# stanfordnlp/mac-network

Hardware: NVIDIA H100
Metric: mac_reasoning_steps_per_sec (higher is better)
Workload: dtype bf16

## Files before the change

mac_network_b200/csrc/read_step.cuh:

```cuda
#pragma once
#include "tc_gemm.cuh"

namespace mac {

constexpr int RS_D = 512;
constexpr int RS_BM = 64;
constexpr int RS_KB = RS_D / TC_BK;
constexpr int RS_BLK = RS_BM * TC_BK * 2;
constexpr int RS_A_BYTES = RS_KB * RS_BLK;
constexpr int RS_B_HALF = 256 * TC_BK * 2;
constexpr int RS_CONSUMERS = 256;
constexpr int RS_THREADS = RS_CONSUMERS + 32;

constexpr int RS128_BM = 128;
constexpr int RS128_BLK = RS128_BM * TC_BK * 2;
constexpr int RS128_A_BYTES = RS_KB * RS128_BLK;
constexpr int RS128_STAGE = RS_B_HALF;
constexpr int RS128_STAGES = 3;
constexpr int RS128_Q0 = RS_KB;
constexpr int RS128_G1B = RS128_Q0 + 2;
constexpr int RS128_Q1 = RS128_G1B + RS_KB;
constexpr int RS128_G2A = RS128_Q1 + 2;
constexpr int RS128_G2B = RS128_G2A + RS_KB;
constexpr int RS128_SLOTS = RS128_G2B + RS_KB;
constexpr int RS128_CONSUMERS = 256;
constexpr int RS128_THREADS = RS128_CONSUMERS + 128;
constexpr int RS128_SMEM_BYTES = RS128_A_BYTES + RS128_STAGES * RS128_STAGE + 1024  +
                                 8 * (RS_KB + 2 * RS128_STAGES) ;
static_assert(RS128_SMEM_BYTES <= 232448, "over the sm_90 per-block shared memory opt-in limit");
static_assert(RS128_BLK % 1024 == 0 && RS128_STAGE % 1024 == 0 && (RS128_BM / 2) * 128 % 1024 == 0,
              "swizzled operands need 1024-byte alignment");
static_assert(2 * RS128_BLK == RS128_STAGE, "a ring slot holds two Q blocks");
constexpr int RS128_PRODUCER_REGS = 40;
constexpr int RS128_CONSUMER_REGS = 232;
static_assert(RS128_PRODUCER_REGS + 2 * RS128_CONSUMER_REGS <= 3 * (65536 / RS128_THREADS / 8 * 8), "register budget");

__device__ __forceinline__ float bf16lo(uint32_t w) { return __uint_as_float(w << 16); }
__device__ __forceinline__ float bf16hi(uint32_t w) { return __uint_as_float(w & 0xffff0000u); }

__device__ __forceinline__ void wgmma_bf16_n256(float (&d)[128], uint64_t adesc, uint64_t bdesc, uint32_t accum) {
  asm volatile(
      "{\n\t.reg .pred p;\n\t"
      "setp.ne.b32 p, %130, 0;\n\t"
      "wgmma.mma_async.sync.aligned.m64n256k16.f32.bf16.bf16 "
      "{%0, %1, %2, %3, %4, %5, %6, %7, %8, %9, %10, %11, %12, %13, %14, %15, %16, %17, %18, %19, %20, %21, %22, %23, %24, %25, %26, %27, %28, %29, %30, %31, %32, %33, %34, %35, %36, %37, %38, %39, %40, %41, %42, %43, %44, %45, %46, %47, %48, %49, %50, %51, %52, %53, %54, %55, %56, %57, %58, %59, %60, %61, %62, %63, %64, %65, %66, %67, %68, %69, %70, %71, %72, %73, %74, %75, %76, %77, %78, %79, %80, %81, %82, %83, %84, %85, %86, %87, %88, %89, %90, %91, %92, %93, %94, %95, %96, %97, %98, %99, %100, %101, %102, %103, %104, %105, %106, %107, %108, %109, %110, %111, %112, %113, %114, %115, %116, %117, %118, %119, %120, %121, %122, %123, %124, %125, %126, %127}, %128, %129, p, 1, 1, 0, 0;\n\t}"
      : "+f"(d[0]), "+f"(d[1]), "+f"(d[2]), "+f"(d[3]), "+f"(d[4]), "+f"(d[5]), "+f"(d[6]), "+f"(d[7]), "+f"(d[8]), "+f"(d[9]), "+f"(d[10]), "+f"(d[11]), "+f"(d[12]), "+f"(d[13]), "+f"(d[14]), "+f"(d[15]), "+f"(d[16]), "+f"(d[17]), "+f"(d[18]), "+f"(d[19]), "+f"(d[20]), "+f"(d[21]), "+f"(d[22]), "+f"(d[23]), "+f"(d[24]), "+f"(d[25]), "+f"(d[26]), "+f"(d[27]), "+f"(d[28]), "+f"(d[29]), "+f"(d[30]), "+f"(d[31]), "+f"(d[32]), "+f"(d[33]), "+f"(d[34]), "+f"(d[35]), "+f"(d[36]), "+f"(d[37]), "+f"(d[38]), "+f"(d[39]), "+f"(d[40]), "+f"(d[41]), "+f"(d[42]), "+f"(d[43]), "+f"(d[44]), "+f"(d[45]), "+f"(d[46]), "+f"(d[47]), "+f"(d[48]), "+f"(d[49]), "+f"(d[50]), "+f"(d[51]), "+f"(d[52]), "+f"(d[53]), "+f"(d[54]), "+f"(d[55]), "+f"(d[56]), "+f"(d[57]), "+f"(d[58]), "+f"(d[59]), "+f"(d[60]), "+f"(d[61]), "+f"(d[62]), "+f"(d[63]), "+f"(d[64]), "+f"(d[65]), "+f"(d[66]), "+f"(d[67]), "+f"(d[68]), "+f"(d[69]), "+f"(d[70]), "+f"(d[71]), "+f"(d[72]), "+f"(d[73]), "+f"(d[74]), "+f"(d[75]), "+f"(d[76]), "+f"(d[77]), "+f"(d[78]), "+f"(d[79]), "+f"(d[80]), "+f"(d[81]), "+f"(d[82]), "+f"(d[83]), "+f"(d[84]), "+f"(d[85]), "+f"(d[86]), "+f"(d[87]), "+f"(d[88]), "+f"(d[89]), "+f"(d[90]), "+f"(d[91]), "+f"(d[92]), "+f"(d[93]), "+f"(d[94]), "+f"(d[95]), "+f"(d[96]), "+f"(d[97]), "+f"(d[98]), "+f"(d[99]), "+f"(d[100]), "+f"(d[101]), "+f"(d[102]), "+f"(d[103]), "+f"(d[104]), "+f"(d[105]), "+f"(d[106]), "+f"(d[107]), "+f"(d[108]), "+f"(d[109]), "+f"(d[110]), "+f"(d[111]), "+f"(d[112]), "+f"(d[113]), "+f"(d[114]), "+f"(d[115]), "+f"(d[116]), "+f"(d[117]), "+f"(d[118]), "+f"(d[119]), "+f"(d[120]), "+f"(d[121]), "+f"(d[122]), "+f"(d[123]), "+f"(d[124]), "+f"(d[125]), "+f"(d[126]), "+f"(d[127])
      : "l"(adesc), "l"(bdesc), "r"(accum));
}
inline bool read_step_supported(int B, int N, int d) {
  return d == RS_D && N >= 1 && N <= 256 && B >= 1 && B < (1 << 22);
}

struct ReadStepParams {
  int M, N;
  const float* y;
  const float* ctrl;
  const float* bm2;
  const float* wr;
  float* logits;
};

__device__ __forceinline__ void rs_consumer_bar() { asm volatile("bar.sync 1, %0;" ::"n"(RS_CONSUMERS) : "memory"); }

__device__ __forceinline__ void rs128_wg_bar(int g) { asm volatile("bar.sync %0, 128;" ::"r"(1 + g) : "memory"); }

__device__ __forceinline__ void rs128_gemm_half(float (&acc)[128], uint32_t a_u, uint32_t ring_u, uint64_t* full,
                                                uint64_t* empty, int t0, int lane) {
  for (int j = 0; j < RS_KB; ++j) {
    const int t = t0 + j, s = t % RS128_STAGES;
    mbar_wait(&full[s], (t / RS128_STAGES) & 1);
    const uint64_t adesc = make_sw128_kmajor_desc(a_u + j * RS128_BLK);
    const uint64_t bdesc = make_sw128_kmajor_desc(ring_u + s * RS128_STAGE);
    wgmma_fence();
#pragma unroll
    for (int k = 0; k < TC_BK / 16; ++k) wgmma_bf16_n256(acc, adesc + 2 * k, bdesc + 2 * k, (j || k) ? 1u : 0u);
    wgmma_commit();
    wgmma_wait<1>();
    wgmma_hold(acc);
    if (j && lane == 0) mbar_arrive(&empty[(t - 1) % RS128_STAGES]);
  }
  wgmma_wait<0>();
  wgmma_hold(acc);
  if (lane == 0) mbar_arrive(&empty[(t0 + RS_KB - 1) % RS128_STAGES]);
}

__device__ __forceinline__ int rs128_sw_off(int r, int n, int blk) {
  return (n >> 6) * blk + r * 128 + ((((n & 63) >> 3) ^ (r & 7)) << 4) + (n & 7) * 2;
}

__global__ void __launch_bounds__(RS128_THREADS, 1)
read_step_kernel(const __grid_constant__ CUtensorMap map_p, const __grid_constant__ CUtensorMap map_q,
                 const __grid_constant__ CUtensorMap map_w1, const __grid_constant__ CUtensorMap map_w2,
                 const ReadStepParams p) {
  extern __shared__ unsigned char smem_dyn[];
  const uint32_t base_u32 = smem_u32(smem_dyn);
  unsigned char* a_tile = smem_dyn + ((1024u - (base_u32 & 1023u)) & 1023u);
  unsigned char* ring = a_tile + RS128_A_BYTES;
  uint64_t* pfull = reinterpret_cast<uint64_t*>(ring + RS128_STAGES * RS128_STAGE);
  uint64_t* full = pfull + RS_KB;
  uint64_t* empty = full + RS128_STAGES;

  const int warp = threadIdx.x >> 5, lane = threadIdx.x & 31;
  const int row0 = blockIdx.x * RS128_BM;

  if (threadIdx.x == RS128_CONSUMERS) {
    tma_prefetch_desc(&map_p);
    tma_prefetch_desc(&map_q);
    tma_prefetch_desc(&map_w1);
    tma_prefetch_desc(&map_w2);
    for (int i = 0; i < RS_KB; ++i) mbar_init(&pfull[i], 1);
    for (int i = 0; i < RS128_STAGES; ++i) {
      mbar_init(&full[i], 1);
      mbar_init(&empty[i], RS128_CONSUMERS / 32);
    }
    fence_mbar_init();
  }
  __syncthreads();

  if (warp >= RS128_CONSUMERS / 32) {
    asm volatile("setmaxnreg.dec.sync.aligned.u32 %0;" ::"n"(RS128_PRODUCER_REGS));
    if (warp == RS128_CONSUMERS / 32 && elect_one()) {
      auto load_p = [&](int j) {
        mbar_expect_tx(&pfull[j], RS128_BLK);
        tma_load_2d(a_tile + j * RS128_BLK, &map_p, j * TC_BK, row0, &pfull[j]);
      };
      for (int t = 0; t < RS128_SLOTS; ++t) {
        if (t < RS128_STAGES) load_p(t);
        else if (t == RS128_STAGES)
          for (int j = RS128_STAGES; j < RS_KB; ++j) load_p(j);
        const int s = t % RS128_STAGES;
        mbar_wait(&empty[s], ((t / RS128_STAGES) & 1) ^ 1);
        unsigned char* dst = ring + s * RS128_STAGE;
        mbar_expect_tx(&full[s], RS128_STAGE);
        if (t < RS128_G2A) {
          const int half = t >= RS128_G1B, u = t - half * RS128_G1B;
          if (u < RS_KB) {
            tma_load_2d(dst, &map_w1, u * TC_BK, 256 * half, &full[s]);
          } else {
            const int kb = 4 * half + 2 * (u - RS_KB);
            tma_load_2d(dst, &map_q, kb * TC_BK, row0, &full[s]);
            tma_load_2d(dst + RS128_BLK, &map_q, (kb + 1) * TC_BK, row0, &full[s]);
          }
        } else {
          const int half = t >= RS128_G2B, u = t - (half ? RS128_G2B : RS128_G2A);
          tma_load_2d(dst, &map_w2, u * TC_BK, 256 * half, &full[s]);
        }
      }
    }
    return;
  }

  asm volatile("setmaxnreg.inc.sync.aligned.u32 %0;" ::"n"(RS128_CONSUMER_REGS));
  const int g = warp >> 2;
  const int wt = threadIdx.x & 127;
  const int rl = 16 * (warp & 3) + (lane >> 2);
  const int cq = 2 * (lane & 3);
  const int rowg = row0 + 64 * g;
  unsigned char* a_wg = a_tile + g * (RS128_BM / 2) * 128;
  const uint32_t a_u = smem_u32(a_wg), ring_u = smem_u32(ring);
  const int prow = wt >> 3;
  const int poff = prow * 128 + (wt & 7) * 16;
  const int pcol = ((wt & 7) ^ (prow & 7)) << 3;
  int yoff[4];
#pragma unroll
  for (int u = 0; u < 4; ++u) yoff[u] = min(rowg + prow + 16 * u, p.M - 1) / p.N * RS_D + pcol;

  float acc[128];
  float4 y0[4], y1[4];
  auto load_y = [&](int j) {
#pragma unroll
    for (int u = 0; u < 4; ++u) {
      y0[u] = *reinterpret_cast<const float4*>(p.y + yoff[u] + j * TC_BK);
      y1[u] = *reinterpret_cast<const float4*>(p.y + yoff[u] + j * TC_BK + 4);
    }
  };
  load_y(0);
  for (int j = 0; j < RS_KB; ++j) {
    const int s = j % RS128_STAGES;
    mbar_wait(&pfull[j], 0);
#pragma unroll
    for (int u = 0; u < 4; ++u) {
      uint4* c = reinterpret_cast<uint4*>(a_wg + j * RS128_BLK + poff + u * 16 * 128);
      const uint4 v = *c;
      *c = make_uint4(pack_bf16(bf16lo(v.x) * y0[u].x, bf16hi(v.x) * y0[u].y), pack_bf16(bf16lo(v.y) * y0[u].z, bf16hi(v.y) * y0[u].w),
                      pack_bf16(bf16lo(v.z) * y1[u].x, bf16hi(v.z) * y1[u].y), pack_bf16(bf16lo(v.w) * y1[u].z, bf16hi(v.w) * y1[u].w));
    }
    fence_proxy_async();
    rs128_wg_bar(g);
    mbar_wait(&full[s], (j / RS128_STAGES) & 1);
    const uint64_t adesc = make_sw128_kmajor_desc(a_u + j * RS128_BLK);
    const uint64_t bdesc = make_sw128_kmajor_desc(ring_u + s * RS128_STAGE);
    wgmma_fence();
#pragma unroll
    for (int k = 0; k < TC_BK / 16; ++k) wgmma_bf16_n256(acc, adesc + 2 * k, bdesc + 2 * k, (j || k) ? 1u : 0u);
    wgmma_commit();
    if (j + 1 < RS_KB) load_y(j + 1);
    wgmma_wait<1>();
    wgmma_hold(acc);
    if (j && lane == 0) mbar_arrive(&empty[(j - 1) % RS128_STAGES]);
  }
  wgmma_wait<0>();
  wgmma_hold(acc);
  if (lane == 0) mbar_arrive(&empty[(RS_KB - 1) % RS128_STAGES]);

  uint32_t h0[64];
#pragma unroll
  for (int q = 0; q < 2; ++q) {
    const int t = RS128_Q0 + q, s = t % RS128_STAGES;
    mbar_wait(&full[s], (t / RS128_STAGES) & 1);
    const unsigned char* q_tile = ring + s * RS128_STAGE + g * (RS128_BM / 2) * 128 - 2 * q * RS128_BLK;
#pragma unroll
    for (int h = 0; h < 2; ++h) {
      const int r = rl + 8 * h;
      const bool live = rowg + r < p.M;
#pragma unroll
      for (int j = 16 * q; j < 16 * q + 16; ++j) {
        const uint32_t qv = *reinterpret_cast<const uint32_t*>(q_tile + rs128_sw_off(r, cq + 8 * j, RS128_BLK));
        h0[2 * j + h] = live ? pack_bf16(elu_fast(acc[4 * j + 2 * h] + bf16lo(qv)), elu_fast(acc[4 * j + 2 * h + 1] + bf16hi(qv)))
                             : 0u;
      }
    }
    __syncwarp();
    if (lane == 0) mbar_arrive(&empty[s]);
  }

  rs128_gemm_half(acc, a_u, ring_u, full, empty, RS128_G1B, lane);

  rs128_wg_bar(g);
#pragma unroll
  for (int h = 0; h < 2; ++h) {
    const int r = rl + 8 * h;
#pragma unroll
    for (int j = 0; j < 32; ++j) *reinterpret_cast<uint32_t*>(a_wg + rs128_sw_off(r, cq + 8 * j, RS128_BLK)) = h0[2 * j + h];
  }
#pragma unroll
  for (int q = 0; q < 2; ++q) {
    const int t = RS128_Q1 + q, s = t % RS128_STAGES;
    mbar_wait(&full[s], (t / RS128_STAGES) & 1);
    const unsigned char* q_tile = ring + s * RS128_STAGE + g * (RS128_BM / 2) * 128 - 2 * q * RS128_BLK;
#pragma unroll
    for (int h = 0; h < 2; ++h) {
      const int r = rl + 8 * h;
      const bool live = rowg + r < p.M;
#pragma unroll
      for (int j = 16 * q; j < 16 * q + 16; ++j) {
        const int n = cq + 8 * j;
        const uint32_t qv = *reinterpret_cast<const uint32_t*>(q_tile + rs128_sw_off(r, n, RS128_BLK));
        *reinterpret_cast<uint32_t*>(a_wg + rs128_sw_off(r, 256 + n, RS128_BLK)) =
            live ? pack_bf16(elu_fast(acc[4 * j + 2 * h] + bf16lo(qv)), elu_fast(acc[4 * j + 2 * h + 1] + bf16hi(qv))) : 0u;
      }
    }
    __syncwarp();
    if (lane == 0) mbar_arrive(&empty[s]);
  }
  fence_proxy_async();
  rs128_wg_bar(g);

  float part[2][2];
#pragma unroll
  for (int half = 0; half < 2; ++half) {
    rs128_gemm_half(acc, a_u, ring_u, full, empty, half ? RS128_G2B : RS128_G2A, lane);
#pragma unroll
    for (int h = 0; h < 2; ++h) {
      const int row = rowg + rl + 8 * h;
      const float* crow = p.ctrl + (size_t)(min(row, p.M - 1) / p.N) * RS_D + 256 * half;
      const float* bm2 = p.bm2 + 256 * half;
      const float* wr = p.wr + 256 * half;
      float s = 0.f;
#pragma unroll
      for (int j = 0; j < 32; ++j) {
        const int n = cq + 8 * j;
        const float2 cc = __ldg(reinterpret_cast<const float2*>(crow + n));
        const float2 bb = __ldg(reinterpret_cast<const float2*>(bm2 + n));
        const float2 ww = __ldg(reinterpret_cast<const float2*>(wr + n));
        const float t0 = elu_fast((acc[4 * j + 2 * h] + bb.x) * cc.x);
        const float t1 = elu_fast((acc[4 * j + 2 * h + 1] + bb.y) * cc.y);
        s = fmaf(t0, ww.x, s);
        s = fmaf(t1, ww.y, s);
      }
      s += __shfl_xor_sync(0xffffffffu, s, 1);
      s += __shfl_xor_sync(0xffffffffu, s, 2);
      part[half][h] = s;
    }
  }
#pragma unroll
  for (int h = 0; h < 2; ++h) {
    const int row = rowg + rl + 8 * h;
    if ((lane & 3) == 0 && row < p.M) p.logits[row] = part[0][h] + part[1][h];
  }
}

inline int read_step_launch(const void* P, const void* Q, float* logits, const void* kb_bf16, const float* y,
                            const float* control, const mac_read_weights* w, float* att, float* info, int B, int N, int d,
                            cudaStream_t stream) {
  const int M = B * N;
  CUtensorMap mp, mq, mw1, mw2;
  int st = make_tmap_2d(&mp, P, 1, (uint64_t)M, (uint64_t)d, (uint64_t)d * 2, RS128_BM, TC_BK, 1);
  if (st != MAC_OK) return st;
  st = make_tmap_2d(&mq, Q, 1, (uint64_t)M, (uint64_t)d, (uint64_t)d * 2, RS128_BM, TC_BK, 1);
  if (st != MAC_OK) return st;
  st = make_tmap_2d(&mw1, w->Wm_bf16, 1, (uint64_t)d, (uint64_t)d, (uint64_t)2 * d * 2, 256, TC_BK, 1);
  if (st != MAC_OK) return st;
  st = make_tmap_2d(&mw2, w->Wm2_bf16, 1, (uint64_t)d, (uint64_t)d, (uint64_t)d * 2, 256, TC_BK, 1);
  if (st != MAC_OK) return st;
  ReadStepParams p{};
  p.M = M; p.N = N; p.y = y; p.ctrl = control; p.bm2 = w->bm2; p.wr = w->wr; p.logits = logits;
  MAC_CUDA_TRY(cudaFuncSetAttribute(read_step_kernel, cudaFuncAttributeMaxDynamicSharedMemorySize, RS128_SMEM_BYTES));
  read_step_kernel<<<(M + RS128_BM - 1) / RS128_BM, RS128_THREADS, RS128_SMEM_BYTES, stream>>>(mp, mq, mw1, mw2, p);
  MAC_LAUNCH_CHECK();
  return mac_kb_attend_fwd(logits, 1, w->br, kb_bf16, 1, att, info, B, N, d, stream);
}

}
```

profiles/read_step_128.py:

```python
import argparse
import json
import os
import shutil
import subprocess
import sys
import tempfile

import numpy as np

ROOT = os.path.dirname(os.path.dirname(os.path.abspath(__file__)))
LIB_REL = os.path.join("mac_network_b200", "csrc", "libmac_b200.so")
SIDES = ("base", "new")


def device_info():
    q = subprocess.run(["nvidia-smi", "--query-gpu=name,power.limit,clocks.max.sm", "--format=csv,noheader"],
                       capture_output=True, text=True, timeout=60)
    name, power, clock = [s.strip() for s in q.stdout.strip().splitlines()[0].split(",")]
    return {"name": name, "power_limit": power, "max_sm_clock": clock}


def spread(xs):
    xs = [float(x) for x in xs]
    return {"median": float(np.median(xs)), "min": min(xs), "max": max(xs), "runs": [round(x, 3) for x in xs]}


def tree_copy(dst, lib):
    shutil.copytree(ROOT, dst, ignore=shutil.ignore_patterns(".git", "*.o", "__pycache__"))
    shutil.copyfile(lib, os.path.join(dst, LIB_REL))
    return dst


def bench(tree, extra, timeout_s=1800):
    out = subprocess.run([sys.executable, os.path.join(tree, "bench.py")] + extra, capture_output=True, text=True,
                         timeout=timeout_s, cwd=tree)
    if out.returncode != 0:
        raise RuntimeError("bench.py %s: exit %d: %s" % (" ".join(extra), out.returncode, out.stderr[-2000:]))
    line = json.loads(out.stdout.strip().splitlines()[-1])
    print("%s %s: %s" % (os.path.basename(tree), " ".join(extra), line.get("value", "done")), flush=True)
    return line


def main():
    ap = argparse.ArgumentParser()
    ap.add_argument("out_dir")
    ap.add_argument("--base-lib", required=True)
    ap.add_argument("--runs", type=int, default=3)
    ap.add_argument("--roof-runs", type=int, default=6)
    ap.add_argument("--part", default="both", choices=["rooflines", "headline", "both"])
    args = ap.parse_args()
    out = {"device": device_info(), "runs": args.runs, "roof_runs": args.roof_runs,
           "headline_args": "--gpus 1 --steps 480 --warmup 12 --skip-cpu"}
    tmp = tempfile.mkdtemp(prefix="read_step_128_")
    try:
        trees = {"base": tree_copy(os.path.join(tmp, "base"), os.path.abspath(args.base_lib)),
                 "new": tree_copy(os.path.join(tmp, "new"), os.path.join(ROOT, LIB_REL))}
        dumps = {s: os.path.join(tmp, "dump_" + s) for s in SIDES}

        roof = {s: [] for s in SIDES}
        for _ in range(args.roof_runs if args.part != "headline" else 0):
            for s in SIDES:
                roof[s].append(bench(trees[s], ["--rooflines-only"])["read_step_fused"]["us"])
        if args.part != "headline":
            out["read_step_fused_us"] = {s: spread(roof[s]) for s in SIDES}
            out["read_step_fused_speedup"] = (out["read_step_fused_us"]["base"]["median"] /
                                              out["read_step_fused_us"]["new"]["median"])
        if args.part == "rooflines":
            return finish(args, out)

        lines = {s: {"headline": [], "bf16_gqa": [], "batched_one_stream": [], "batched_two_streams": []} for s in SIDES}
        for i in range(args.runs):
            for s in SIDES:
                extra = ["--gpus", "1", "--steps", "480", "--warmup", "12", "--skip-cpu"]
                line = bench(trees[s], extra + (["--dump-outputs", dumps[s]] if i == 0 else []))
                lines[s]["headline"].append(line["value"])
                lines[s]["bf16_gqa"].append(line["sub_lines"]["bf16_gqa"]["value"])
                lines[s]["batched_one_stream"].append(line["info_batched_requests"]["requests_x6_one_stream"]["value"])
                lines[s]["batched_two_streams"].append(line["info_batched_requests"]["requests_x6_two_streams"]["value"])
        out["reasoning_steps_per_s"] = {s: {k: spread(v) for k, v in lines[s].items()} for s in SIDES}
        out["headline_speedup"] = (out["reasoning_steps_per_s"]["new"]["headline"]["median"] /
                                   out["reasoning_steps_per_s"]["base"]["headline"]["median"])

        same = {}
        for name in sorted(os.listdir(dumps["base"])):
            a, b = np.load(os.path.join(dumps["base"], name)), np.load(os.path.join(dumps["new"], name))
            same[name] = bool(a.shape == b.shape and a.dtype == b.dtype and a.tobytes() == b.tobytes())
        out["outputs_bit_identical"] = same
    finally:
        shutil.rmtree(tmp, ignore_errors=True)
    finish(args, out)


def finish(args, out):
    os.makedirs(args.out_dir, exist_ok=True)
    path = os.path.join(args.out_dir, "read_step_128_%s_h100.json" % args.part)
    with open(path, "w") as f:
        json.dump(out, f, indent=1)
    print(json.dumps(out))


if __name__ == "__main__":
    main()
```

Measured before the change: 19460.

## Split read-step first GEMM into N=128 quarters and overlap epilogue with next quarter

Splits the first GEMM of the fused read-step kernel into four N=128 quarters, held in two 64-register accumulators used in ping-pong. The ELU(acc+Q) epilogue of each quarter runs while the next quarter's wgmma is in flight, instead of running only after the full N=256 halves finish. The TMA ring is rebuilt as six 128-row slots, with Q blocks interleaved into the weight stream, and the second GEMM still issues N=256 by pairing adjacent slots. This adds more barrier traffic, narrower wgmma shapes in GEMM1, and higher register pressure from holding three quarters of bf16 h values.

```diff
diff --git a/mac_network_b200/csrc/read_step.cuh b/mac_network_b200/csrc/read_step.cuh
--- a/mac_network_b200/csrc/read_step.cuh
+++ b/mac_network_b200/csrc/read_step.cuh
@@ -8,21 +8,20 @@
 constexpr int RS_KB = RS_D / TC_BK;
 constexpr int RS_BLK = RS_BM * TC_BK * 2;
 constexpr int RS_A_BYTES = RS_KB * RS_BLK;
-constexpr int RS_B_HALF = 256 * TC_BK * 2;
 constexpr int RS_CONSUMERS = 256;
 constexpr int RS_THREADS = RS_CONSUMERS + 32;
 
 constexpr int RS128_BM = 128;
 constexpr int RS128_BLK = RS128_BM * TC_BK * 2;
 constexpr int RS128_A_BYTES = RS_KB * RS128_BLK;
-constexpr int RS128_STAGE = RS_B_HALF;
-constexpr int RS128_STAGES = 3;
-constexpr int RS128_Q0 = RS_KB;
-constexpr int RS128_G1B = RS128_Q0 + 2;
-constexpr int RS128_Q1 = RS128_G1B + RS_KB;
-constexpr int RS128_G2A = RS128_Q1 + 2;
-constexpr int RS128_G2B = RS128_G2A + RS_KB;
-constexpr int RS128_SLOTS = RS128_G2B + RS_KB;
+constexpr int RS128_QN = 128;
+constexpr int RS128_STAGE = RS128_QN * TC_BK * 2;
+constexpr int RS128_STAGES = 6;
+constexpr int RS128_G1Q = RS_KB;
+constexpr int RS128_G1Q_SLOTS = RS_KB + 2;
+constexpr int RS128_Q3 = RS128_G1Q + 3 * RS128_G1Q_SLOTS;
+constexpr int RS128_G2 = RS128_Q3 + 2;
+constexpr int RS128_SLOTS = RS128_G2 + 4 * RS_KB;
 constexpr int RS128_CONSUMERS = 256;
 constexpr int RS128_THREADS = RS128_CONSUMERS + 128;
 constexpr int RS128_SMEM_BYTES = RS128_A_BYTES + RS128_STAGES * RS128_STAGE + 1024  +
@@ -30,7 +29,20 @@
 static_assert(RS128_SMEM_BYTES <= 232448, "over the sm_90 per-block shared memory opt-in limit");
 static_assert(RS128_BLK % 1024 == 0 && RS128_STAGE % 1024 == 0 && (RS128_BM / 2) * 128 % 1024 == 0,
               "swizzled operands need 1024-byte alignment");
-static_assert(2 * RS128_BLK == RS128_STAGE, "a ring slot holds two Q blocks");
+static_assert(RS128_BLK == RS128_STAGE, "a ring slot holds one Q block");
+static_assert(4 * RS128_QN == RS_D && RS128_QN == 2 * TC_BK, "four quarters of two Q blocks each");
+static_assert(RS128_STAGES >= 4, "a held Q slot leaves 3 or more weight slots in flight");
+
+__host__ __device__ constexpr int rs128_g1_slot(int q, int j) {
+  return q == 0 ? j : RS128_G1Q + (q - 1) * RS128_G1Q_SLOTS + 1 + j + (j >= 2);
+}
+__host__ __device__ constexpr int rs128_q_slot(int q, int b) {
+  return q < 3 ? RS128_G1Q + q * RS128_G1Q_SLOTS + 3 * b : RS128_Q3 + b;
+}
+__host__ __device__ constexpr int rs128_g2_slot(int h, int j) { return RS128_G2 + 2 * (h * RS_KB + j); }
+static_assert(rs128_q_slot(0, 0) + 1 == rs128_g1_slot(1, 0) && rs128_q_slot(0, 1) + 1 == rs128_g1_slot(1, 2) &&
+              rs128_g1_slot(3, RS_KB - 1) + 1 == rs128_q_slot(3, 0) && rs128_q_slot(3, 1) + 1 == rs128_g2_slot(0, 0) &&
+              rs128_g2_slot(1, RS_KB - 1) + 2 == RS128_SLOTS && RS128_G2 % 2 == 0 && RS128_STAGES % 2 == 0, "ring slot order");
 constexpr int RS128_PRODUCER_REGS = 40;
 constexpr int RS128_CONSUMER_REGS = 232;
 static_assert(RS128_PRODUCER_REGS + 2 * RS128_CONSUMER_REGS <= 3 * (65536 / RS128_THREADS / 8 * 8), "register budget");
@@ -38,13 +50,14 @@
 __device__ __forceinline__ float bf16lo(uint32_t w) { return __uint_as_float(w << 16); }
 __device__ __forceinline__ float bf16hi(uint32_t w) { return __uint_as_float(w & 0xffff0000u); }
 
-__device__ __forceinline__ void wgmma_bf16_n256(float (&d)[128], uint64_t adesc, uint64_t bdesc, uint32_t accum) {
+__device__ __forceinline__ void wgmma_bf16_n256(float (&lo)[64], float (&hi)[64], uint64_t adesc, uint64_t bdesc,
+                                                uint32_t accum) {
   asm volatile(
       "{\n\t.reg .pred p;\n\t"
       "setp.ne.b32 p, %130, 0;\n\t"
       "wgmma.mma_async.sync.aligned.m64n256k16.f32.bf16.bf16 "
       "{%0, %1, %2, %3, %4, %5, %6, %7, %8, %9, %10, %11, %12, %13, %14, %15, %16, %17, %18, %19, %20, %21, %22, %23, %24, %25, %26, %27, %28, %29, %30, %31, %32, %33, %34, %35, %36, %37, %38, %39, %40, %41, %42, %43, %44, %45, %46, %47, %48, %49, %50, %51, %52, %53, %54, %55, %56, %57, %58, %59, %60, %61, %62, %63, %64, %65, %66, %67, %68, %69, %70, %71, %72, %73, %74, %75, %76, %77, %78, %79, %80, %81, %82, %83, %84, %85, %86, %87, %88, %89, %90, %91, %92, %93, %94, %95, %96, %97, %98, %99, %100, %101, %102, %103, %104, %105, %106, %107, %108, %109, %110, %111, %112, %113, %114, %115, %116, %117, %118, %119, %120, %121, %122, %123, %124, %125, %126, %127}, %128, %129, p, 1, 1, 0, 0;\n\t}"
-      : "+f"(d[0]), "+f"(d[1]), "+f"(d[2]), "+f"(d[3]), "+f"(d[4]), "+f"(d[5]), "+f"(d[6]), "+f"(d[7]), "+f"(d[8]), "+f"(d[9]), "+f"(d[10]), "+f"(d[11]), "+f"(d[12]), "+f"(d[13]), "+f"(d[14]), "+f"(d[15]), "+f"(d[16]), "+f"(d[17]), "+f"(d[18]), "+f"(d[19]), "+f"(d[20]), "+f"(d[21]), "+f"(d[22]), "+f"(d[23]), "+f"(d[24]), "+f"(d[25]), "+f"(d[26]), "+f"(d[27]), "+f"(d[28]), "+f"(d[29]), "+f"(d[30]), "+f"(d[31]), "+f"(d[32]), "+f"(d[33]), "+f"(d[34]), "+f"(d[35]), "+f"(d[36]), "+f"(d[37]), "+f"(d[38]), "+f"(d[39]), "+f"(d[40]), "+f"(d[41]), "+f"(d[42]), "+f"(d[43]), "+f"(d[44]), "+f"(d[45]), "+f"(d[46]), "+f"(d[47]), "+f"(d[48]), "+f"(d[49]), "+f"(d[50]), "+f"(d[51]), "+f"(d[52]), "+f"(d[53]), "+f"(d[54]), "+f"(d[55]), "+f"(d[56]), "+f"(d[57]), "+f"(d[58]), "+f"(d[59]), "+f"(d[60]), "+f"(d[61]), "+f"(d[62]), "+f"(d[63]), "+f"(d[64]), "+f"(d[65]), "+f"(d[66]), "+f"(d[67]), "+f"(d[68]), "+f"(d[69]), "+f"(d[70]), "+f"(d[71]), "+f"(d[72]), "+f"(d[73]), "+f"(d[74]), "+f"(d[75]), "+f"(d[76]), "+f"(d[77]), "+f"(d[78]), "+f"(d[79]), "+f"(d[80]), "+f"(d[81]), "+f"(d[82]), "+f"(d[83]), "+f"(d[84]), "+f"(d[85]), "+f"(d[86]), "+f"(d[87]), "+f"(d[88]), "+f"(d[89]), "+f"(d[90]), "+f"(d[91]), "+f"(d[92]), "+f"(d[93]), "+f"(d[94]), "+f"(d[95]), "+f"(d[96]), "+f"(d[97]), "+f"(d[98]), "+f"(d[99]), "+f"(d[100]), "+f"(d[101]), "+f"(d[102]), "+f"(d[103]), "+f"(d[104]), "+f"(d[105]), "+f"(d[106]), "+f"(d[107]), "+f"(d[108]), "+f"(d[109]), "+f"(d[110]), "+f"(d[111]), "+f"(d[112]), "+f"(d[113]), "+f"(d[114]), "+f"(d[115]), "+f"(d[116]), "+f"(d[117]), "+f"(d[118]), "+f"(d[119]), "+f"(d[120]), "+f"(d[121]), "+f"(d[122]), "+f"(d[123]), "+f"(d[124]), "+f"(d[125]), "+f"(d[126]), "+f"(d[127])
+      : "+f"(lo[0]), "+f"(lo[1]), "+f"(lo[2]), "+f"(lo[3]), "+f"(lo[4]), "+f"(lo[5]), "+f"(lo[6]), "+f"(lo[7]), "+f"(lo[8]), "+f"(lo[9]), "+f"(lo[10]), "+f"(lo[11]), "+f"(lo[12]), "+f"(lo[13]), "+f"(lo[14]), "+f"(lo[15]), "+f"(lo[16]), "+f"(lo[17]), "+f"(lo[18]), "+f"(lo[19]), "+f"(lo[20]), "+f"(lo[21]), "+f"(lo[22]), "+f"(lo[23]), "+f"(lo[24]), "+f"(lo[25]), "+f"(lo[26]), "+f"(lo[27]), "+f"(lo[28]), "+f"(lo[29]), "+f"(lo[30]), "+f"(lo[31]), "+f"(lo[32]), "+f"(lo[33]), "+f"(lo[34]), "+f"(lo[35]), "+f"(lo[36]), "+f"(lo[37]), "+f"(lo[38]), "+f"(lo[39]), "+f"(lo[40]), "+f"(lo[41]), "+f"(lo[42]), "+f"(lo[43]), "+f"(lo[44]), "+f"(lo[45]), "+f"(lo[46]), "+f"(lo[47]), "+f"(lo[48]), "+f"(lo[49]), "+f"(lo[50]), "+f"(lo[51]), "+f"(lo[52]), "+f"(lo[53]), "+f"(lo[54]), "+f"(lo[55]), "+f"(lo[56]), "+f"(lo[57]), "+f"(lo[58]), "+f"(lo[59]), "+f"(lo[60]), "+f"(lo[61]), "+f"(lo[62]), "+f"(lo[63]), "+f"(hi[0]), "+f"(hi[1]), "+f"(hi[2]), "+f"(hi[3]), "+f"(hi[4]), "+f"(hi[5]), "+f"(hi[6]), "+f"(hi[7]), "+f"(hi[8]), "+f"(hi[9]), "+f"(hi[10]), "+f"(hi[11]), "+f"(hi[12]), "+f"(hi[13]), "+f"(hi[14]), "+f"(hi[15]), "+f"(hi[16]), "+f"(hi[17]), "+f"(hi[18]), "+f"(hi[19]), "+f"(hi[20]), "+f"(hi[21]), "+f"(hi[22]), "+f"(hi[23]), "+f"(hi[24]), "+f"(hi[25]), "+f"(hi[26]), "+f"(hi[27]), "+f"(hi[28]), "+f"(hi[29]), "+f"(hi[30]), "+f"(hi[31]), "+f"(hi[32]), "+f"(hi[33]), "+f"(hi[34]), "+f"(hi[35]), "+f"(hi[36]), "+f"(hi[37]), "+f"(hi[38]), "+f"(hi[39]), "+f"(hi[40]), "+f"(hi[41]), "+f"(hi[42]), "+f"(hi[43]), "+f"(hi[44]), "+f"(hi[45]), "+f"(hi[46]), "+f"(hi[47]), "+f"(hi[48]), "+f"(hi[49]), "+f"(hi[50]), "+f"(hi[51]), "+f"(hi[52]), "+f"(hi[53]), "+f"(hi[54]), "+f"(hi[55]), "+f"(hi[56]), "+f"(hi[57]), "+f"(hi[58]), "+f"(hi[59]), "+f"(hi[60]), "+f"(hi[61]), "+f"(hi[62]), "+f"(hi[63])
       : "l"(adesc), "l"(bdesc), "r"(accum));
 }
 inline bool read_step_supported(int B, int N, int d) {
@@ -64,24 +77,26 @@
 
 __device__ __forceinline__ void rs128_wg_bar(int g) { asm volatile("bar.sync %0, 128;" ::"r"(1 + g) : "memory"); }
 
-__device__ __forceinline__ void rs128_gemm_half(float (&acc)[128], uint32_t a_u, uint32_t ring_u, uint64_t* full,
-                                                uint64_t* empty, int t0, int lane) {
-  for (int j = 0; j < RS_KB; ++j) {
-    const int t = t0 + j, s = t % RS128_STAGES;
-    mbar_wait(&full[s], (t / RS128_STAGES) & 1);
-    const uint64_t adesc = make_sw128_kmajor_desc(a_u + j * RS128_BLK);
-    const uint64_t bdesc = make_sw128_kmajor_desc(ring_u + s * RS128_STAGE);
-    wgmma_fence();
-#pragma unroll
-    for (int k = 0; k < TC_BK / 16; ++k) wgmma_bf16_n256(acc, adesc + 2 * k, bdesc + 2 * k, (j || k) ? 1u : 0u);
-    wgmma_commit();
-    wgmma_wait<1>();
-    wgmma_hold(acc);
-    if (j && lane == 0) mbar_arrive(&empty[(t - 1) % RS128_STAGES]);
-  }
-  wgmma_wait<0>();
+__device__ __forceinline__ void rs128_zero(float (&acc)[64]) {
+#pragma unroll
+  for (int i = 0; i < 64; ++i) acc[i] = 0.f;
+}
+
+template <typename F>
+__device__ __forceinline__ void rs128_kblock(float (&acc)[64], uint32_t a_u, uint32_t ring_u, uint64_t* full,
+                                             uint64_t* empty, int j, int t, int tp, int lane, F&& issued) {
+  const int s = t % RS128_STAGES;
+  mbar_wait(&full[s], (t / RS128_STAGES) & 1);
+  const uint64_t adesc = make_sw128_kmajor_desc(a_u + j * RS128_BLK);
+  const uint64_t bdesc = make_sw128_kmajor_desc(ring_u + s * RS128_STAGE);
+  wgmma_fence();
+#pragma unroll
+  for (int k = 0; k < TC_BK / 16; ++k) wgmma_bf16_n128(acc, adesc + 2 * k, bdesc + 2 * k, (j || k) ? 1u : 0u);
+  wgmma_commit();
+  issued();
+  wgmma_wait<1>();
   wgmma_hold(acc);
-  if (lane == 0) mbar_arrive(&empty[(t0 + RS_KB - 1) % RS128_STAGES]);
+  if (tp >= 0 && lane == 0) mbar_arrive(&empty[tp % RS128_STAGES]);
 }
 
 __device__ __forceinline__ int rs128_sw_off(int r, int n, int blk) {
@@ -124,28 +139,30 @@
         mbar_expect_tx(&pfull[j], RS128_BLK);
         tma_load_2d(a_tile + j * RS128_BLK, &map_p, j * TC_BK, row0, &pfull[j]);
       };
-      for (int t = 0; t < RS128_SLOTS; ++t) {
+      int t = 0;
+      auto put = [&](const CUtensorMap* map, int kb, int y0) {
         if (t < RS128_STAGES) load_p(t);
         else if (t == RS128_STAGES)
           for (int j = RS128_STAGES; j < RS_KB; ++j) load_p(j);
         const int s = t % RS128_STAGES;
         mbar_wait(&empty[s], ((t / RS128_STAGES) & 1) ^ 1);
-        unsigned char* dst = ring + s * RS128_STAGE;
         mbar_expect_tx(&full[s], RS128_STAGE);
-        if (t < RS128_G2A) {
-          const int half = t >= RS128_G1B, u = t - half * RS128_G1B;
-          if (u < RS_KB) {
-            tma_load_2d(dst, &map_w1, u * TC_BK, 256 * half, &full[s]);
-          } else {
-            const int kb = 4 * half + 2 * (u - RS_KB);
-            tma_load_2d(dst, &map_q, kb * TC_BK, row0, &full[s]);
-            tma_load_2d(dst + RS128_BLK, &map_q, (kb + 1) * TC_BK, row0, &full[s]);
-          }
-        } else {
-          const int half = t >= RS128_G2B, u = t - (half ? RS128_G2B : RS128_G2A);
-          tma_load_2d(dst, &map_w2, u * TC_BK, 256 * half, &full[s]);
+        tma_load_2d(ring + s * RS128_STAGE, map, kb * TC_BK, y0, &full[s]);
+        ++t;
+      };
+      for (int j = 0; j < RS_KB; ++j) put(&map_w1, j, 0);
+      for (int q = 1; q < 4; ++q)
+        for (int j = 0; j < RS_KB; ++j) {
+          if (j == 0 || j == 2) put(&map_q, 2 * (q - 1) + j / 2, row0);
+          put(&map_w1, j, RS128_QN * q);
         }
-      }
+      put(&map_q, RS_KB - 2, row0);
+      put(&map_q, RS_KB - 1, row0);
+      for (int h = 0; h < 2; ++h)
+        for (int j = 0; j < RS_KB; ++j) {
+          put(&map_w2, j, 2 * RS128_QN * h);
+          put(&map_w2, j, 2 * RS128_QN * h + RS128_QN);
+        }
     }
     return;
   }
@@ -165,7 +182,7 @@
 #pragma unroll
   for (int u = 0; u < 4; ++u) yoff[u] = min(rowg + prow + 16 * u, p.M - 1) / p.N * RS_D + pcol;
 
-  float acc[128];
+  float accA[64], accB[64];
   float4 y0[4], y1[4];
   auto load_y = [&](int j) {
 #pragma unroll
@@ -176,7 +193,6 @@
   };
   load_y(0);
   for (int j = 0; j < RS_KB; ++j) {
-    const int s = j % RS128_STAGES;
     mbar_wait(&pfull[j], 0);
 #pragma unroll
     for (int u = 0; u < 4; ++u) {
@@ -187,71 +203,67 @@
     }
     fence_proxy_async();
     rs128_wg_bar(g);
-    mbar_wait(&full[s], (j / RS128_STAGES) & 1);
-    const uint64_t adesc = make_sw128_kmajor_desc(a_u + j * RS128_BLK);
-    const uint64_t bdesc = make_sw128_kmajor_desc(ring_u + s * RS128_STAGE);
-    wgmma_fence();
-#pragma unroll
-    for (int k = 0; k < TC_BK / 16; ++k) wgmma_bf16_n256(acc, adesc + 2 * k, bdesc + 2 * k, (j || k) ? 1u : 0u);
-    wgmma_commit();
-    if (j + 1 < RS_KB) load_y(j + 1);
-    wgmma_wait<1>();
-    wgmma_hold(acc);
-    if (j && lane == 0) mbar_arrive(&empty[(j - 1) % RS128_STAGES]);
-  }
+    rs128_kblock(accA, a_u, ring_u, full, empty, j, rs128_g1_slot(0, j), j ? rs128_g1_slot(0, j - 1) : -1, lane, [&] {
+      if (j + 1 < RS_KB) load_y(j + 1);
+    });
+  }
+
+  auto epi1 = [&](const float (&acc)[64], uint32_t (&h)[32], int q, int j) {
+    const int t = rs128_q_slot(q, j >> 1), s = t % RS128_STAGES;
+    if (!(j & 1)) mbar_wait(&full[s], (t / RS128_STAGES) & 1);
+    const unsigned char* q_tile = ring + s * RS128_STAGE + g * (RS128_BM / 2) * 128;
+#pragma unroll
+    for (int hh = 0; hh < 2; ++hh) {
+      const int r = rl + 8 * hh;
+      const uint32_t live = rowg + r < p.M ? 0xffffffffu : 0u;
+#pragma unroll
+      for (int i = 4 * j; i < 4 * j + 4; ++i) {
+        const uint32_t qv = *reinterpret_cast<const uint32_t*>(q_tile + rs128_sw_off(r, cq + 8 * (i & 7), RS128_BLK));
+        h[2 * i + hh] = live & pack_bf16(elu_fast(acc[4 * i + 2 * hh] + bf16lo(qv)), elu_fast(acc[4 * i + 2 * hh + 1] + bf16hi(qv)));
+      }
+    }
+    if (j & 1) {
+      __syncwarp();
+      if (lane == 0) mbar_arrive(&empty[s]);
+    }
+  };
+  auto store_h = [&](const uint32_t (&h)[32], int q) {
+#pragma unroll
+    for (int hh = 0; hh < 2; ++hh) {
+      const int r = rl + 8 * hh;
+#pragma unroll
+      for (int i = 0; i < 16; ++i)
+        *reinterpret_cast<uint32_t*>(a_wg + rs128_sw_off(r, RS128_QN * q + cq + 8 * i, RS128_BLK)) = h[2 * i + hh];
+    }
+  };
+
+  uint32_t hreg[3][32];
+  auto g1_quarter = [&](float (&acc)[64], float (&prev)[64], uint32_t (&h)[32], int q) {
+    rs128_zero(acc);
+#pragma unroll
+    for (int j = 0; j < RS_KB; ++j) {
+      rs128_kblock(acc, a_u, ring_u, full, empty, j, rs128_g1_slot(q, j), rs128_g1_slot(j ? q : q - 1, (j + RS_KB - 1) % RS_KB),
+                   lane, [] {});
+      if (j == 0) wgmma_hold(prev);
+      if (j < 4) epi1(prev, h, q - 1, j);
+    }
+  };
+  g1_quarter(accB, accA, hreg[0], 1);
+  g1_quarter(accA, accB, hreg[1], 2);
+  g1_quarter(accB, accA, hreg[2], 3);
   wgmma_wait<0>();
-  wgmma_hold(acc);
-  if (lane == 0) mbar_arrive(&empty[(RS_KB - 1) % RS128_STAGES]);
-
-  uint32_t h0[64];
-#pragma unroll
-  for (int q = 0; q < 2; ++q) {
-    const int t = RS128_Q0 + q, s = t % RS128_STAGES;
-    mbar_wait(&full[s], (t / RS128_STAGES) & 1);
-    const unsigned char* q_tile = ring + s * RS128_STAGE + g * (RS128_BM / 2) * 128 - 2 * q * RS128_BLK;
-#pragma unroll
-    for (int h = 0; h < 2; ++h) {
-      const int r = rl + 8 * h;
-      const bool live = rowg + r < p.M;
-#pragma unroll
-      for (int j = 16 * q; j < 16 * q + 16; ++j) {
-        const uint32_t qv = *reinterpret_cast<const uint32_t*>(q_tile + rs128_sw_off(r, cq + 8 * j, RS128_BLK));
-        h0[2 * j + h] = live ? pack_bf16(elu_fast(acc[4 * j + 2 * h] + bf16lo(qv)), elu_fast(acc[4 * j + 2 * h + 1] + bf16hi(qv)))
-                             : 0u;
-      }
-    }
-    __syncwarp();
-    if (lane == 0) mbar_arrive(&empty[s]);
-  }
-
-  rs128_gemm_half(acc, a_u, ring_u, full, empty, RS128_G1B, lane);
+  wgmma_hold(accB);
+  if (lane == 0) mbar_arrive(&empty[rs128_g1_slot(3, RS_KB - 1) % RS128_STAGES]);
 
   rs128_wg_bar(g);
-#pragma unroll
-  for (int h = 0; h < 2; ++h) {
-    const int r = rl + 8 * h;
-#pragma unroll
-    for (int j = 0; j < 32; ++j) *reinterpret_cast<uint32_t*>(a_wg + rs128_sw_off(r, cq + 8 * j, RS128_BLK)) = h0[2 * j + h];
-  }
-#pragma unroll
-  for (int q = 0; q < 2; ++q) {
-    const int t = RS128_Q1 + q, s = t % RS128_STAGES;
-    mbar_wait(&full[s], (t / RS128_STAGES) & 1);
-    const unsigned char* q_tile = ring + s * RS128_STAGE + g * (RS128_BM / 2) * 128 - 2 * q * RS128_BLK;
-#pragma unroll
-    for (int h = 0; h < 2; ++h) {
-      const int r = rl + 8 * h;
-      const bool live = rowg + r < p.M;
-#pragma unroll
-      for (int j = 16 * q; j < 16 * q + 16; ++j) {
-        const int n = cq + 8 * j;
-        const uint32_t qv = *reinterpret_cast<const uint32_t*>(q_tile + rs128_sw_off(r, n, RS128_BLK));
-        *reinterpret_cast<uint32_t*>(a_wg + rs128_sw_off(r, 256 + n, RS128_BLK)) =
-            live ? pack_bf16(elu_fast(acc[4 * j + 2 * h] + bf16lo(qv)), elu_fast(acc[4 * j + 2 * h + 1] + bf16hi(qv))) : 0u;
-      }
-    }
-    __syncwarp();
-    if (lane == 0) mbar_arrive(&empty[s]);
+  store_h(hreg[0], 0);
+  store_h(hreg[1], 1);
+  store_h(hreg[2], 2);
+  {
+    uint32_t h3[32];
+#pragma unroll
+    for (int j = 0; j < 4; ++j) epi1(accB, h3, 3, j);
+    store_h(h3, 3);
   }
   fence_proxy_async();
   rs128_wg_bar(g);
@@ -259,10 +271,37 @@
   float part[2][2];
 #pragma unroll
   for (int half = 0; half < 2; ++half) {
-    rs128_gemm_half(acc, a_u, ring_u, full, empty, half ? RS128_G2B : RS128_G2A, lane);
-#pragma unroll
-    for (int h = 0; h < 2; ++h) {
-      const int row = rowg + rl + 8 * h;
+    rs128_zero(accA);
+    rs128_zero(accB);
+    for (int j = 0; j < RS_KB; ++j) {
+      const int t = rs128_g2_slot(half, j), s = t % RS128_STAGES;
+      mbar_wait(&full[s], (t / RS128_STAGES) & 1);
+      mbar_wait(&full[s + 1], ((t + 1) / RS128_STAGES) & 1);
+      const uint64_t adesc = make_sw128_kmajor_desc(a_u + j * RS128_BLK);
+      const uint64_t bdesc = make_sw128_kmajor_desc(ring_u + s * RS128_STAGE);
+      wgmma_fence();
+#pragma unroll
+      for (int k = 0; k < TC_BK / 16; ++k) wgmma_bf16_n256(accB, accA, adesc + 2 * k, bdesc + 2 * k, (j || k) ? 1u : 0u);
+      wgmma_commit();
+      wgmma_wait<1>();
+      wgmma_hold(accA);
+      wgmma_hold(accB);
+      if (j && lane == 0) {
+        mbar_arrive(&empty[(t - 2) % RS128_STAGES]);
+        mbar_arrive(&empty[(t - 1) % RS128_STAGES]);
+      }
+    }
+    wgmma_wait<0>();
+    wgmma_hold(accA);
+    wgmma_hold(accB);
+    if (lane == 0) {
+      const int t = rs128_g2_slot(half, RS_KB - 1);
+      mbar_arrive(&empty[t % RS128_STAGES]);
+      mbar_arrive(&empty[(t + 1) % RS128_STAGES]);
+    }
+#pragma unroll
+    for (int hh = 0; hh < 2; ++hh) {
+      const int row = rowg + rl + 8 * hh;
       const float* crow = p.ctrl + (size_t)(min(row, p.M - 1) / p.N) * RS_D + 256 * half;
       const float* bm2 = p.bm2 + 256 * half;
       const float* wr = p.wr + 256 * half;
@@ -273,20 +312,21 @@
         const float2 cc = __ldg(reinterpret_cast<const float2*>(crow + n));
         const float2 bb = __ldg(reinterpret_cast<const float2*>(bm2 + n));
         const float2 ww = __ldg(reinterpret_cast<const float2*>(wr + n));
-        const float t0 = elu_fast((acc[4 * j + 2 * h] + bb.x) * cc.x);
-        const float t1 = elu_fast((acc[4 * j + 2 * h + 1] + bb.y) * cc.y);
+        const float (&acc)[64] = j < 16 ? accB : accA;
+        const float t0 = elu_fast((acc[4 * (j & 15) + 2 * hh] + bb.x) * cc.x);
+        const float t1 = elu_fast((acc[4 * (j & 15) + 2 * hh + 1] + bb.y) * cc.y);
         s = fmaf(t0, ww.x, s);
         s = fmaf(t1, ww.y, s);
-      }
+              }
       s += __shfl_xor_sync(0xffffffffu, s, 1);
       s += __shfl_xor_sync(0xffffffffu, s, 2);
-      part[half][h] = s;
-    }
-  }
-#pragma unroll
-  for (int h = 0; h < 2; ++h) {
-    const int row = rowg + rl + 8 * h;
-    if ((lane & 3) == 0 && row < p.M) p.logits[row] = part[0][h] + part[1][h];
+      part[half][hh] = s;
+    }
+  }
+#pragma unroll
+  for (int hh = 0; hh < 2; ++hh) {
+    const int row = rowg + rl + 8 * hh;
+    if ((lane & 3) == 0 && row < p.M) p.logits[row] = part[0][hh] + part[1][hh];
   }
 }
 
@@ -299,9 +339,9 @@
   if (st != MAC_OK) return st;
   st = make_tmap_2d(&mq, Q, 1, (uint64_t)M, (uint64_t)d, (uint64_t)d * 2, RS128_BM, TC_BK, 1);
   if (st != MAC_OK) return st;
-  st = make_tmap_2d(&mw1, w->Wm_bf16, 1, (uint64_t)d, (uint64_t)d, (uint64_t)2 * d * 2, 256, TC_BK, 1);
+  st = make_tmap_2d(&mw1, w->Wm_bf16, 1, (uint64_t)d, (uint64_t)d, (uint64_t)2 * d * 2, RS128_QN, TC_BK, 1);
   if (st != MAC_OK) return st;
-  st = make_tmap_2d(&mw2, w->Wm2_bf16, 1, (uint64_t)d, (uint64_t)d, (uint64_t)d * 2, 256, TC_BK, 1);
+  st = make_tmap_2d(&mw2, w->Wm2_bf16, 1, (uint64_t)d, (uint64_t)d, (uint64_t)d * 2, RS128_QN, TC_BK, 1);
   if (st != MAC_OK) return st;
   ReadStepParams p{};
   p.M = M; p.N = N; p.y = y; p.ctrl = control; p.bm2 = w->bm2; p.wr = w->wr; p.logits = logits;
diff --git a/profiles/read_step_128.py b/profiles/read_step_128.py
--- a/profiles/read_step_128.py
+++ b/profiles/read_step_128.py
@@ -48,6 +48,7 @@
     ap.add_argument("--runs", type=int, default=3)
     ap.add_argument("--roof-runs", type=int, default=6)
     ap.add_argument("--part", default="both", choices=["rooflines", "headline", "both"])
+    ap.add_argument("--prefix", default="read_step_128", help="output file name prefix")
     args = ap.parse_args()
     out = {"device": device_info(), "runs": args.runs, "roof_runs": args.roof_runs,
            "headline_args": "--gpus 1 --steps 480 --warmup 12 --skip-cpu"}
@@ -93,7 +94,7 @@
 
 def finish(args, out):
     os.makedirs(args.out_dir, exist_ok=True)
-    path = os.path.join(args.out_dir, "read_step_128_%s_h100.json" % args.part)
+    path = os.path.join(args.out_dir, "%s_%s_h100.json" % (args.prefix, args.part))
     with open(path, "w") as f:
         json.dump(out, f, indent=1)
     print(json.dumps(out))
```

Result: no change. 19160, median of 6 (-1.5%).
